# Shanmuk4622/RL-Project-Heist-Architect-Adversarial-Reinforcement-Learning-Framework-CSE4019

Measured on AMD Instinct MI355X. Metric: Solver env-steps/sec at 20×20, 4096 envs/GPU, 1/2/4/8 MI355X, higher is better.
Workload: dtype f64

## Files before the change

rl-project-heist-architect-adversarial-reinforcement-learning-framework-cse4019_amd/csrc/heist_env.hip:

```cpp
#include <type_traits>
#include <utility>

#include "heist_device.h"
#include "heist_fan_intervals.h"
#include "heist_trig.h"

#pragma clang fp contract(off)

namespace heist {

__constant__ double kSinCosTab[4 * HEIST_SINCOS_TAB_ROWS] = HEIST_SINCOS_TAB_INIT;
constexpr int kTabDoubles = 4 * HEIST_SINCOS_TAB_ROWS;

__device__ __forceinline__ int iabs_(int a) { return a < 0 ? -a : a; }
__device__ __forceinline__ int unpack_r(uint16_t v) { return v & 0xff; }
__device__ __forceinline__ int unpack_c(uint16_t v) { return v >> 8; }

__device__ __forceinline__ double py_mod360(double x) {
  if (x > 0.0 && x < 720.0) return x >= 360.0 ? x - 360.0 : x;
  double r = fmod(x, 360.0);
  if (r != 0.0) {
    if (r < 0.0) r += 360.0;
  } else {
    r = 0.0;
// ... 2441 lines not shown
  int hdr[4];
};

constexpr double kFanUnitsPerDeg = 4294967296.0 / 360.0;
struct IvlTable {
  uint32_t cut[kFanCuts];
  float2 dir[kFanCuts];
  uint8_t idx[368];
};
static_assert(sizeof(IvlTable) % 16 == 0, "copied in 16-byte words");
constexpr IvlTable make_ivl_table() {
  IvlTable t{};
  for (int j = 0; j < kFanCuts; ++j) {
    t.cut[j] = kFanCut[j];
    t.dir[j] = float2{kFanDir[j][0], kFanDir[j][1]};
  }
  for (int d = 0; d < 361; ++d) t.idx[d] = kFanIdx[d];
  return t;
}
__constant__ IvlTable kIvlTable = make_ivl_table();
constexpr size_t kLeanUnion = sizeof(LeanStage) > sizeof(IvlTable) ? sizeof(LeanStage) : sizeof(IvlTable);
struct LeanLds {
  uint8_t* grid;
  uint16_t* path;
  uint8_t* act;
  LeanStage* stg;
  IvlTable* ivl;
  uint4* icam;
  int32_t* icim;
  uint16_t* cone;
  uint16_t* rcone;
  uint8_t* gpl;
  float4* plane2;
};
__host__ __device__ constexpr int lean_gap(int R, int C) { return (R + 2 * kRing) * (C + 2 * kRing) <= 1024 ? 1024 : 2048; }
__host__ __device__ inline size_t lean_carve(unsigned char* smem, int R, int C, int mc, int mg, int mp, int K,
                                             LeanLds* L) {
  size_t o = 3 * (size_t)lean_gap(R, C);
  if (L) L->grid = smem + o;
  o += align16((size_t)R * C);
  if (L) L->path = reinterpret_cast<uint16_t*>(smem + o);
  o += align16(2 * (size_t)mg * mp);
  if (L) L->act = smem + o;
  o += align16((size_t)K);
  if (L) L->stg = reinterpret_cast<LeanStage*>(smem + o);
  if (L) L->ivl = reinterpret_cast<IvlTable*>(smem + o);
  o += align16(kLeanUnion);
  if (L) L->icam = reinterpret_cast<uint4*>(smem + o);
  o += 16 * (size_t)(mc > 0 ? mc : 1);
  if (L) L->icim = reinterpret_cast<int32_t*>(smem + o);
  o += align16(8 * (size_t)(mc > 0 ? mc : 1));
  if (L) L->cone = reinterpret_cast<uint16_t*>(smem + o);
  o += 64 * (size_t)(mg > 0 ? mg : 1);
  if (L) L->rcone = reinterpret_cast<uint16_t*>(smem + o);
  o += 64 * (size_t)(mg > 0 ? mg : 1);
  if (L) L->gpl = smem + o;
  o += align16((size_t)R * C);
  if (L) L->plane2 = reinterpret_cast<float4*>(smem + o);
  o += 4 * (size_t)R * C;
  return o;
}
static size_t lean_lds_bytes(const EnvParams& p, int K) {
  const size_t lean = align16(lean_carve(nullptr, p.R, p.C, p.max_cams, p.max_guards, p.max_path, K, nullptr)) +
                      (p.stamps ? 80 : 0);
  const size_t generic = step_multi_lds(p, K);
  return lean > generic ? lean : generic;
}


struct LeanGuard {
  uint32_t a, b, nslot;
  __device__ int idx() const { return (int)(a & 0xffu); }
  __device__ int step() const { return (int)((a >> 8) & 0xffu); }
  __device__ int len() const { return (int)((a >> 16) & 0xffu); }
  __device__ int hslot() const { return (int)(a >> 24); }
  __device__ uint32_t pos() const { return b & 0xffffu; }
  __device__ uint32_t pos0() const { return b >> 16; }
};

template <int D, bool REC>
__device__ __attribute__((noinline)) void lean_generic_body(EnvParams p, int K, const int64_t* __restrict__ actions,
                                                            obs_out_t<REC>* __restrict__ obs, float* __restrict__ rew,
                                                            double* __restrict__ rew64, uint8_t* __restrict__ done_out,
                                                            int8_t* __restrict__ status_out, int auto_reset,
                                                            unsigned char* smem, int e) {
  step_multi_body<1, D, false, 0, REC>(p, K, actions, obs, rew, rew64, done_out, status_out, auto_reset, smem, e);
}

template <int R_, int C_, bool STAMP = false, int NW = 1, bool REC = false>
__global__ __launch_bounds__(64 * NW) __attribute__((amdgpu_waves_per_eu(4))) void step_lean_kernel(
    EnvParams p, int K, const int64_t* __restrict__ actions, obs_out_t<REC>* __restrict__ obs, float* __restrict__ rew,
    double* __restrict__ rew64, uint8_t* __restrict__ done_out, int8_t* __restrict__ status_out, int auto_reset) {
  constexpr int D = lean_gap(R_, C_);
  constexpr int PC = C_ + 2 * kRing;
  constexpr int RC = R_ * C_;
  constexpr int N4 = RC / 4;
  constexpr int C4 = C_ / 4;
  constexpr int Q = (N4 + 63) / 64;
  constexpr int OFF0 = kRing * PC + kRing;
  static_assert((R_ + 2 * kRing) * PC <= D, "the padded planes fit the 1024-byte gap");
  static_assert(C_ % 4 == 0 && R_ <= 64 && C_ <= 32 && (R_ + 2 * kRing) * PC <= 2048, "lean kernel geometry");
  static_assert(NW == 1 || (NW == 2 && !STAMP && Q % 2 == 0), "two waves: the plain form, even Q");
  constexpr int QW = Q / NW;
  static_assert(!REC || !STAMP, "record output: the plain instances only");
  constexpr int NVIS = (RC + 31) / 32;
  constexpr int RW = (NVIS + 1 + 3) & ~3;
  constexpr int kStores = REC ? QW + 1 + 4 : 3 * QW + 4;
  extern __shared__ __align__(16) unsigned char smem[];
  const int e = block_env(p);
  if (p.prio_mode && p.dispatch_order) {
    const int pr = (int)((uint32_t)p.order[blockIdx.x] >> 24);
    if (pr == 3) __builtin_amdgcn_s_setprio(3);
    else if (pr == 2) __builtin_amdgcn_s_setprio(2);
    else if (pr == 1) __builtin_amdgcn_s_setprio(1);
  }
  const int lane = NW == 1 ? (int)threadIdx.x : (int)(threadIdx.x & 63u);
  const int wid = NW == 1 ? 0 : __builtin_amdgcn_readfirstlane((int)(threadIdx.x >> 6));
  const int tid = threadIdx.x;
  const int N = p.n_envs;
  const int mc = p.max_cams, mg = p.max_guards, n_slot = mc + mg, mp = p.max_path;
  const EnvBase eb = env_base(p, e);
  const FanTick* fan0 = p.fan + p.fan_base;

  EnvScalars s = p.scal[e];
  const int g = lane - mc;
  double heading = 0.0, speed = 0.0;
  uint32_t cam_rc = 0;
  LeanGuard gd{0u, 0u, 0u};
  const bool live_cam = lane < s.n_cams, live_guard = g >= 0 && g < s.n_guards;
  bool cached = false;
  double fovd = 0.0, su = 1.0;
  int32_t im_fx = 0;
  int cam_n = 0;
  bool ivl = false;
  {
    EmitterRaw rec;
    rec.a = make_uint4(0u, 0u, 0u, 0u);
    rec.b = rec.a;
    if (lane < n_slot) {
      const uint4* rs = lane < mc ? reinterpret_cast<const uint4*>(eb.cams + (uint32_t)lane)
                                  : reinterpret_cast<const uint4*>(eb.guards + (uint32_t)g);
      rec.a = rs[0];
      rec.b = rs[1];
    }
    const Cam cm = as_cam(rec);
    const Guard gr = as_guard(rec);
    heading = cm.heading;
    speed = cm.speed;
    cam_rc = (uint32_t)cm.row | ((uint32_t)cm.col << 8);
    cached = live_guard && gr.hslot != kUncached;
    gd.a = (uint32_t)(uint8_t)gr.idx | ((uint32_t)(uint8_t)gr.step << 8) | ((uint32_t)(uint8_t)gr.len << 16) |
           ((uint32_t)gr.hslot << 24);
    gd.b = (uint32_t)gr.pos | ((uint32_t)gr.pos0 << 16);
    gd.nslot = gr.nslot;
    const double f_heading = fan0->heading, f_speed = fan0->speed, f_fov = fan0->fov;
    const int f_rays = fan0->num_rays, f_range = fan0->range, f_uniq = fan0->n_uniq;
    const bool cam_ok = !live_cam || (py_mod360(cm.heading + cm.speed * 1.0) == f_heading && cm.speed == f_speed &&
                                      cm.fov == f_fov && cm.num_rays == f_rays && cm.range == f_range);
    const bool base_ok = p.ray_mode == 0 && !s.done && __ballot(live_guard && !cached) == 0ull;
    const bool fan_ok = p.fan_on && f_uniq >= 0 && f_range == kTieMaxRange && __ballot(!cam_ok) == 0ull;
    const double su_ = (cm.fov / (double)cm.num_rays) * kFanUnitsPerDeg;
    const bool ivl_cam = !live_cam || (cm.range == kTieMaxRange && cm.num_rays >= 1 && cm.fov > 0.0 &&
                                       cm.fov < 170.0 && su_ > 2.0 * (double)kFanMarginAxis + 8.0 &&
                                       su_ >= 2097153.0);
    ivl = base_ok && !fan_ok && p.interval_fans && __ballot(!ivl_cam) == 0ull;
    if (!base_ok || (!fan_ok && !ivl)) {
      if (NW == 2 && wid != 0) return;
      lean_generic_body<D, REC>(p, K, actions, obs, rew, rew64, done_out, status_out, auto_reset, smem, e);
      return;
    }
    if (live_cam) {
      fovd = cm.fov;
      su = su_;
      im_fx = (int32_t)__builtin_rint(4503599627370496.0 / su_);
      cam_n = cm.num_rays;
    }
  }

  LeanLds L;
  const size_t carved = lean_carve(smem, R_, C_, mc, mg, mp, K, &L);
  unsigned long long* st_acc = reinterpret_cast<unsigned long long*>(smem + align16(carved));
  unsigned long long st_last = 0, st_start = 0;
  if (STAMP && lane == 0) {
    st_start = st_last = __builtin_amdgcn_s_memtime();
    for (int j = 0; j < 9; ++j) st_acc[j] = 0;
  }
#define LEAN_STAMP(seg)                                        \
  do {                                                         \
    if (STAMP && lane == 0) {                                  \
      const unsigned long long now_ = __builtin_amdgcn_s_memtime(); \
      st_acc[(seg)] += now_ - st_last;                         \
      st_last = now_;                                          \
    }                                                          \
  } while (0)
  uint8_t* const wall = smem;
  uint8_t* const vis = smem + D;
  const uint32_t base = (uint32_t)(uintptr_t)smem;
  const uint32_t stg_a = (uint32_t)__builtin_amdgcn_readfirstlane((int)(uint32_t)(uintptr_t)L.stg);
  const uint32_t stc_a = (uint32_t)__builtin_amdgcn_readfirstlane((int)(uint32_t)(uintptr_t)L.cone);
  const uint32_t str_a = (uint32_t)__builtin_amdgcn_readfirstlane((int)(uint32_t)(uintptr_t)L.rcone);
  const uint32_t gpl_a = (uint32_t)__builtin_amdgcn_readfirstlane((int)(uint32_t)(uintptr_t)L.gpl);
  static_assert(RC % 16 == 0, "the packed guard plane is cleared in 16-byte words");
  {
    const uint32_t* g4 = reinterpret_cast<const uint32_t*>(p.grid + (size_t)e * RC);
    for (int i = tid; i < N4; i += 64 * NW) reinterpret_cast<uint32_t*>(L.grid)[i] = g4[i];
    const uint8_t* ss = p.stop + (size_t)e * p.stop_bytes;
    for (int i = tid; i < p.stop_bytes; i += 64 * NW) expand_stop(wall, i, ss[i]);
    const int vault = p.vr * C_ + p.vc, qv = vault >> 2;
    for (int q = tid; q < N4; q += 64 * NW) {
      float4 v = reinterpret_cast<const float4*>(p.plane0)[q];
      if (q == qv) patch4(v, vault & 3, p.vault_val);
      L.plane2[q] = v;
    }
  }
  for (int i = tid; i < mg * mp; i += 64 * NW) L.path[i] = eb.paths[i];
  for (int k = tid; k < K; k += 64 * NW) {
    const int64_t a = actions[(size_t)k * N + e];
    L.act[k] = (uint8_t)((a < 0 || a > 4) ? 0 : a);
  }
  __syncthreads();
  uint32_t vwall = 0;
  if (lane < R_)
    for (int c = 0; c < C_; ++c) vwall |= (uint32_t)wall[OFF0 + lane * PC + c] << c;

  auto dma_fan = [&](int k, bool wide) {
    const FanTick* f = fan0 + k;
    lds_dma16(f->off4 + lane, stg_a + (uint32_t)offsetof(LeanStage, off4));
    if (wide) lds_dma16(f->off4 + 64 + lane, stg_a + (uint32_t)offsetof(LeanStage, off4) + 1024u);
    lds_dma16(f->off2 + 2 * lane, stg_a + (uint32_t)offsetof(LeanStage, off2));
    if (lane == 0) lds_dma16(&f->num_rays, stg_a + (uint32_t)offsetof(LeanStage, hdr));
  };
  auto dma_cone = [&](int idx, int slot, uint32_t stage, int par) {
    if (cached) {
      const uint16_t* src = eb.cones + cone_off((uint32_t)g, (uint32_t)idx, (uint32_t)slot);
      const uint32_t dst = stage + (uint32_t)(par * 32 * mg) - 16u * (uint32_t)mc;
      lds_dma16(src, dst);
      lds_dma16(src + 8, dst + 16u * (uint32_t)mg);
    }
  };
  auto dma_next_cone = [&](int par) {
    int idx = gd.idx(), slot = gd.hslot();
    if (gd.len() >= 2) {
      idx += gd.step();
      if (idx >= gd.len()) idx -= gd.len();
      slot = (int)gd.nslot;
    }
    dma_cone(idx, slot, stc_a, par);
    if (auto_reset) dma_cone(0, slot, str_a, par);
  };
  if (wid == 0) dma_next_cone(0);
  if (ivl) {
    for (uint32_t o = 1024u * (uint32_t)wid; o < (uint32_t)sizeof(IvlTable); o += 1024u * NW)
      if (o + 16u * (uint32_t)lane < (uint32_t)sizeof(IvlTable))
        lds_dma16(reinterpret_cast<const unsigned char*>(&kIvlTable) + o + 16u * (uint32_t)lane, stg_a + o);
  } else if (wid == 0) {
    dma_fan(0, true);
  }
  asm volatile("s_waitcnt vmcnt(0)" ::: "memory");
  if (NW == 2) __syncthreads();

  const uint64_t cmask = __ballot(cached);
  auto stamp_cones = [&](const uint16_t* rows, int par) {
    if (lane < RC / 16) reinterpret_cast<uint4*>(L.gpl)[lane] = make_uint4(0u, 0u, 0u, 0u);
    const uint32_t gposv = gd.pos();
    for (int pass = 0; pass * 4 < mg; ++pass) {
      const int i = lane / 15, j = lane - 15 * i;
      const int gs = 4 * pass + i;
      const uint32_t gp = (uint32_t)__shfl((int)gposv, mc + (gs < mg ? gs : 0), 64);
      if (lane < 60 && gs < mg && ((cmask >> (mc + gs)) & 1u)) {
        const uint32_t bits = rows[par * 16 * mg + (j >> 3) * 8 * mg + 8 * gs + (j & 7)] & 0x7fffu;
        if (bits) {
          const uint32_t a0 = gpl_a + (unpack_r((uint16_t)gp) + j - kConeRange) * C_ +
                              (unpack_c((uint16_t)gp) - kConeRange);
          const uint32_t m = bits << (a0 & 3u);
          const uint32_t a = a0 & ~3u;
#pragma unroll
          for (int w = 0; w < 5; ++w) {
            const uint32_t nib = (m >> (4 * w)) & 15u;
            if (nib)
              __hip_atomic_fetch_or(reinterpret_cast<__attribute__((address_space(3))) uint32_t*>(a + 4 * w),
                                    __umul24(nib, 0x204081u) & 0x01010101u, __ATOMIC_RELAXED,
                                    __HIP_MEMORY_SCOPE_WORKGROUP);
          }
        }
      }
    }
  };
  auto march = [&](uint32_t corner, uint4 o4, uint2 o2) {
    const uint32_t ow[6] = {o4.x, o4.y, o4.z, o4.w, o2.x, o2.y};
    uint32_t a[12], w[12];
#pragma unroll
    for (int u = 0; u < 12; ++u) a[u] = corner + ((u & 1) ? (ow[u >> 1] >> 16) : (ow[u >> 1] & 0xffffu));
#pragma unroll
    for (int u = 0; u < 12; ++u) w[u] = lds_ld(a[u]);
    const uint32_t own0 = (ow[0] & 0xffffu) == (uint32_t)OFF0, own1 = (ow[0] >> 16) == (uint32_t)OFF0;
    uint32_t stop = 0;
#pragma unroll
    for (int u = 0; u < 12; ++u) {
      stop = u == 0 ? w[0] : or_b32(stop, w[u]);
      const uint32_t skip = u == 0 ? or_b32(stop, own0) : (u == 1 ? or_b32(stop, own1) : stop);
      lds_st(__umul24(skip, (uint32_t)D) + a[u] + D, 1);
    }
  };
  auto cast_fan = [&](int k, int n_uniq, int n_tie, int par, bool staged_wide) {
#pragma unroll
    for (int z = 0; z < D / 1024; ++z)
      reinterpret_cast<uint4*>(vis)[lane + 64 * z] = make_uint4(0u, 0u, 0u, 0u);
    const FanTick* f = fan0 + k;
    uint4 o4a = make_uint4(0u, 0u, 0u, 0u), o4b = o4a;
    uint2 o2a = make_uint2(0u, 0u), o2b = o2a;
    if (s.n_cams > 0) {
      const bool want_b = n_uniq > 64;
      o4a = L.stg->off4[lane];
      o2a = L.stg->off2[lane];
      if (want_b && staged_wide) {
        o4b = L.stg->off4[64 + lane];
        o2b = L.stg->off2[64 + lane];
      }
      if (want_b && !staged_wide) {
        o4b = f->off4[64 + lane];
        o2b = f->off2[64 + lane];
        asm volatile("" ::"v"(__builtin_bit_cast(u32x4_t, o4a)), "v"(__builtin_bit_cast(u32x2_t, o2a)),
                     "v"(__builtin_bit_cast(u32x4_t, o4b)), "v"(__builtin_bit_cast(u32x2_t, o2b)));
      }
    }
    if (k + 1 < K) {
      asm volatile("s_waitcnt lgkmcnt(0)" ::"v"(__builtin_bit_cast(u32x4_t, o4a)), "v"(__builtin_bit_cast(u32x2_t, o2a)),
                   "v"(__builtin_bit_cast(u32x4_t, o4b)), "v"(__builtin_bit_cast(u32x2_t, o2b))
                   : "memory");
      dma_fan(k + 1, n_uniq > 64);
    }
    if (s.n_cams > 0) {
      for (int m = 0; m < s.n_cams; ++m) {
        const uint32_t rcm = (uint32_t)__builtin_amdgcn_readlane((int)cam_rc, m);
        const uint32_t corner = base + (rcm & 0xffu) * PC + (rcm >> 8);
        if (lane < n_uniq) march(corner, o4a, o2a);
        if (lane + 64 < n_uniq) march(corner, o4b, o2b);
        for (int c0 = 128; c0 < n_uniq; c0 += 64)
          if (lane + c0 < n_uniq) march(corner, f->off4[lane + c0], f->off2[lane + c0]);
      }
      if (n_tie > 0) lean_tie_rays<D, PC>(smem, f, n_tie, cam_rc, s.n_cams, p.half_deg);
    }
    LEAN_STAMP(2);
    stamp_cones(L.cone, par);
  };
  auto wave_join = [&]() {
    if constexpr (NW == 2) asm volatile("s_waitcnt lgkmcnt(0)\n\ts_barrier" ::: "memory");
  };
  auto cast_ivl = [&](int par) {
    wave_join();
#pragma unroll
    for (int z = wid; z < D / 1024; z += NW)
      reinterpret_cast<uint4*>(vis)[lane + 64 * z] = make_uint4(0u, 0u, 0u, 0u);
    const double hmh = heading - fovd / 2.0;
    const double hu = (hmh < 0.0 ? hmh + 360.0 : hmh) * kFanUnitsPerDeg;
    const uint32_t h0v = hu >= 4294967295.0 ? 0xFFFFFFFFu : (uint32_t)hu;
    int cnt = 0, jb = 0;
    if (live_cam) {
      jb = (int)L.ivl->idx[__umulhi(h0v, 360u)] - 1;
      const uint64_t e64 = (uint64_t)h0v + (uint64_t)((double)cam_n * su) + (uint64_t)(kFanMarginAxis + 4);
      const int je = (int)L.ivl->idx[__umulhi((uint32_t)e64, 360u) + 1u] + kFanCuts * (int)(e64 >> 32);
      cnt = je - jb;
      L.icam[lane] = make_uint4(h0v, (uint32_t)jb, (uint32_t)cam_n | (cam_rc << 16), 0u);
      L.icim[lane] = im_fx;
    }
    int total = 0, jo_l = 0, end_l = 0;
    for (int m = 0; m < s.n_cams; ++m) {
      if (lane == m) jo_l = jb - total;
      total += __builtin_amdgcn_readlane(cnt, m);
      if (lane == m) end_l = total;
    }
    auto march_at = [&](uint32_t rc, float2 d) {
      const uint32_t row = rc & 0xffu, col = rc >> 8;
      const uint32_t own = base + (row + kRing) * PC + col + kRing;
      const float mx = __builtin_bit_cast(float, base + col + kRing), my = __builtin_bit_cast(float, row + kRing);
      march_fast<D, 2 * kTieMaxRange, false, false, true>(PC, own, d.x, d.y, mx, my, 2 * kTieMaxRange);
    };
    int mb = 0;
    wave_join();
    for (int q0 = 64 * wid; q0 < total; q0 += 64 * NW) {
      const int q = q0 + lane;
      while (__builtin_amdgcn_readlane(end_l, mb) <= q0) ++mb;
      int c = mb, jo = __builtin_amdgcn_readlane(jo_l, mb);
      for (int m = mb; m + 1 < s.n_cams; ++m) {
        const int em = __builtin_amdgcn_readlane(end_l, m);
        if (em >= q0 + 64) break;
        const int jo_m = __builtin_amdgcn_readlane(jo_l, m + 1);
        if (q >= em) {
          c = m + 1;
          jo = jo_m;
        }
      }
      int j = jo + q;
      j = j < 0 ? j + kFanCuts : (j >= kFanCuts ? j - kFanCuts : j);
      const uint4 cu = L.icam[c];
      const int im = L.icim[c];
      const int n = (int)(cu.z & 0xffffu);
      const int jn = j + 1 == kFanCuts ? 0 : j + 1;
      const uint32_t cut = L.ivl->cut[j], cutn = L.ivl->cut[jn];
      const float2 dj = L.ivl->dir[j];
      const int rel = (int)(cut - cu.x), reln = (int)(cutn - cu.x);
      const int mj = (cut & 0x3FFFFFFFu) ? kFanMarginTie : kFanMarginAxis;
      const int mn = (cutn & 0x3FFFFFFFu) ? kFanMarginTie : kFanMarginAxis;
      const int A = (__mulhi(rel + mj, im) >> 20) + 1;
      const int B = -(__mulhi(mj - rel, im) >> 20);
      const int Bn = -(__mulhi(mn - reln, im) >> 20);
      const int a0 = A > 0 ? A : 0;
      const bool act = q < total;
      const bool safe = act && a0 <= n && a0 < Bn;
      const bool near = act && B < A && B >= 0 && B <= n;
      if (__ballot(near)) {
        const double h_c = __shfl(hmh, c, 64), f_c = __shfl(fovd, c, 64);
        ivl_tie_rays<D, PC>(smem, near ? B : -1, h_c, f_c, n, cu.z >> 16, p.half_deg);
      }
      if (safe) march_at(cu.z >> 16, dj);
    }
    LEAN_STAMP(2);
    if (wid == 0) stamp_cones(L.cone, par);
    wave_join();
  };
  auto cast = [&](int k, int n_uniq, int n_tie, int par, bool staged_wide) {
    if (ivl) {
      cast_ivl(par);
    } else {
      wave_join();
      if (wid == 0) cast_fan(k, n_uniq, n_tie, par, staged_wide);
      wave_join();
    }
  };
  auto read_v1 = [&](uint32_t (&v1)[QW]) {
#pragma unroll
    for (int j = 0; j < QW; ++j) {
      const int q = lane + 64 * (wid * QW + j), qc = q < N4 ? q : N4 - 1, r = qc / C4;
      v1[j] = *reinterpret_cast<const uint32_t*>(vis + OFF0 + r * PC + 4 * (qc - r * C4)) |
              *reinterpret_cast<const uint32_t*>(L.gpl + 4 * qc);
    }
  };

  constexpr uint32_t kOOB = 0x40000000u;
  uint32_t vact = 0;
  bool wide = true;
  for (int k = 0; k < K; ++k) {
    const int par = k & 1;
    if ((k & 63) == 0) vact = k + lane < K ? L.act[k + lane] : 0u;
    asm volatile("s_waitcnt vmcnt(%0)" ::"i"(kStores) : "memory");
    int n_uniq = 0, n_tie = 0;
    if (!ivl && wid == 0) {
      const int2 h = *reinterpret_cast<const int2*>(&L.stg->hdr[2]);
      n_uniq = __builtin_amdgcn_readfirstlane(h.x);
      n_tie = __builtin_amdgcn_readfirstlane(h.y);
    }
    LEAN_STAMP(0);
    const bool staged_wide = wide;
    const bool frozen = s.done != 0;
    double reward = 0.0;
    int status = kAlreadyDone, curr = 0;
    if (!frozen) {
      const int a = __builtin_amdgcn_readlane((int)vact, k & 63);
      const int nr = s.pos_r + (a == 1 ? -1 : (a == 2 ? 1 : 0)), nc = s.pos_c + (a == 3 ? -1 : (a == 4 ? 1 : 0));
      if (nr >= 0 && nr < R_ && nc >= 0 && nc < C_ && !((__builtin_amdgcn_readlane((int)vwall, nr) >> nc) & 1)) {
        s.pos_r = nr;
        s.pos_c = nc;
      }
      status = kRunning;
      curr = iabs_(s.pos_r - p.vr) + iabs_(s.pos_c - p.vc);
      reward = p.r_step;
      reward += (double)(s.prev_dist - curr) * 0.1;
      if (curr <= 3 && s.initial_dist > 3) reward += 0.05 * (double)(3 - curr);
      s.prev_dist = curr;
      if (live_cam) heading = py_mod360(heading + speed * 1.0);
      if (live_guard && gd.len() >= 2) {
        int nidx = gd.idx() + gd.step();
        if (nidx >= gd.len()) nidx -= gd.len();
        const uint32_t np = L.path[__umul24((uint32_t)g, (uint32_t)mp) + (uint32_t)nidx];
        gd.a = (uint32_t)nidx | (gd.a & 0x00ffff00u) | (gd.nslot << 24);
        gd.b = np | (gd.b & 0xffff0000u);
      }
      if (cached && wid == 0) gd.nslot = L.cone[par * 16 * mg + 8 * mg + 8 * g + 7];
      if (k + 1 < K && wid == 0) dma_next_cone(par ^ 1);
      LEAN_STAMP(1);
      cast(k, n_uniq, n_tie, par, staged_wide);
      LEAN_STAMP(3);
    }
    wide = n_uniq > 64;
    uint32_t v1[QW];
    read_v1(v1);
    int done_now = s.done;
    LEAN_STAMP(4);
    if (!frozen) {
      bool seen;
      if constexpr (NW == 1) {
        const int sol = s.pos_r * C_ + s.pos_c, qs = sol >> 2;
        uint32_t vq = v1[0];
#pragma unroll
        for (int j = 1; j < Q; ++j) vq = (qs >> 6) == j ? v1[j] : vq;
        const uint32_t qv = (uint32_t)__builtin_amdgcn_readlane((int)vq, qs & 63);
        seen = ((qv >> (8 * (sol & 3))) & 0xffu) != 0u;
      } else {
        seen = (vis[OFF0 + s.pos_r * PC + s.pos_c] | L.gpl[s.pos_r * C_ + s.pos_c]) != 0;
      }
      if (seen) {
        s.detected = 1;
        reward += p.r_detect;
        s.done = 1;
        status = kDetected;
      }
      if (s.pos_r == p.vr && s.pos_c == p.vc) {
        s.vault_reached = 1;
        reward += p.r_vault;
        s.done = 1;
        status = kVaultReached;
      }
      s.tick += 1;
      if (s.tick >= p.max_steps) {
        s.done = 1;
        status = kTimeout;
        double frac = 1.0 - (double)curr / (double)(s.initial_dist > 1 ? s.initial_dist : 1);
        if (frac < 0.0) frac = 0.0;
        reward += frac * 2.0;
      }
      done_now = s.done;
    }
    LEAN_STAMP(5);
    if (auto_reset && done_now) {
      const bool moved = __ballot(live_guard && gd.pos() != gd.pos0()) != 0ull;
      reset_solver(p, s);
      if (live_guard) {
        gd.a &= ~0xffu;
        gd.b = (gd.b & 0xffff0000u) | gd.pos0();
      }
      if (cached && wid == 0) gd.nslot = L.rcone[par * 16 * mg + 8 * mg + 8 * g + 7];
      if (moved) {
        wave_join();
        if (wid == 0) stamp_cones(L.rcone, par);
        wave_join();
        read_v1(v1);
      }
      if (k + 1 < K && wid == 0) dma_next_cone(par ^ 1);
    }
    LEAN_STAMP(6);
    asm volatile("" ::: "memory");
    if constexpr (REC) {
      uint32_t* o = obs + ((size_t)k * N + e) * RW;
      const __amdgpu_buffer_rsrc_t rs = __builtin_amdgcn_make_buffer_rsrc(o, (short)0, 4 * RW, 0x00020000);
#pragma unroll
      for (int j = 0; j < QW; ++j) {
        const int q = lane + 64 * (wid * QW + j);
        uint32_t w = (q < N4 ? vis_nibble(v1[j]) : 0u) << (4 * (lane & 7));
        w = or8_lanes(w);
        const int wi = q >> 3;
        __builtin_amdgcn_raw_buffer_store_b32(w, rs, (lane & 7) == 0 && wi < NVIS ? 4 * wi : (int)kOOB, 0, 0);
      }
      __builtin_amdgcn_raw_buffer_store_b32(lane == 0 ? (uint32_t)s.pos_r | ((uint32_t)s.pos_c << 8) : 0u, rs,
                                            wid == 0 && lane < RW - NVIS ? 4 * (NVIS + lane) : (int)kOOB, 0, 0);
    } else {
      constexpr int pol = 2;
      float* o = obs + ((size_t)k * N + e) * 3 * RC;
      const __amdgpu_buffer_rsrc_t rs = __builtin_amdgcn_make_buffer_rsrc(o, (short)0, 12 * RC, 0x00020000);
      const int sol = s.pos_r * C_ + s.pos_c, qs = sol >> 2;
      const int vault = p.vr * C_ + p.vc;
  #pragma unroll
      for (int j = 0; j < QW; ++j) {
        const int q = lane + 64 * (wid * QW + j);
        const bool in = q < N4;
        const int qc = in ? q : N4 - 1;
        const uint32_t b = *reinterpret_cast<const uint32_t*>(L.grid + 4 * qc);
        obs_put(rs, pol, in ? 16 * q : (int)kOOB,
                make_float4((float)(b & 0xff) * 0.2f, (float)((b >> 8) & 0xff) * 0.2f,
                            (float)((b >> 16) & 0xff) * 0.2f, (float)(b >> 24) * 0.2f));
        const uint32_t v = v1[j];
        obs_put(rs, pol, in ? 16 * (N4 + q) : (int)kOOB,
                make_float4((float)(v & 0xff), (float)((v >> 8) & 0xff), (float)((v >> 16) & 0xff), (float)(v >> 24)));
        float4 c2 = L.plane2[qc];
        const bool pl = q == qs && sol != vault;
        const int m = sol & 3;
        c2.x = pl && m == 0 ? 1.0f + c2.x : c2.x;
        c2.y = pl && m == 1 ? 1.0f + c2.y : c2.y;
        c2.z = pl && m == 2 ? 1.0f + c2.z : c2.z;
        c2.w = pl && m == 3 ? 1.0f + c2.w : c2.w;
        obs_put(rs, pol, in ? 16 * (2 * N4 + q) : (int)kOOB, c2);
      }
    }
    const uint32_t ko = (uint32_t)((size_t)k * N + e);
    const int l0 = lane == 0 && wid == 0 ? 0 : (int)kOOB;
    __builtin_amdgcn_raw_buffer_store_b32(__builtin_bit_cast(uint32_t, (float)reward),
                                          __builtin_amdgcn_make_buffer_rsrc(rew + ko, (short)0, 4, 0x00020000), l0, 0, 0);
    __builtin_amdgcn_raw_buffer_store_b64(__builtin_bit_cast(u32x2_t, __builtin_bit_cast(uint64_t, reward)),
                                          __builtin_amdgcn_make_buffer_rsrc(rew64 ? rew64 + ko : rew64, (short)0,
                                                                            rew64 ? 8 : 0, 0x00020000),
                                          l0, 0, 0);
    __builtin_amdgcn_raw_buffer_store_b8((uint8_t)done_now,
                                         __builtin_amdgcn_make_buffer_rsrc(done_out + ko, (short)0, 1, 0x00020000), l0,
                                         0, 0);
    __builtin_amdgcn_raw_buffer_store_b8((uint8_t)(int8_t)status,
                                         __builtin_amdgcn_make_buffer_rsrc(status_out + ko, (short)0, 1, 0x00020000),
                                         l0, 0, 0);
    LEAN_STAMP(7);
  }
  if (STAMP && lane == 0) {
    unsigned long long* q = p.stamps + (size_t)e * p.multi_waves * 16;
    for (int j = 0; j < 9; ++j) q[j] = st_acc[j];
    q[9] = __builtin_amdgcn_s_memtime() - st_start;
    q[10] = st_start;
    q[11] = (unsigned)__builtin_amdgcn_s_getreg((31 << 11) | 4);
    q[12] = (unsigned)__builtin_amdgcn_s_getreg((31 << 11) | 20);
  }
#undef LEAN_STAMP
  if (wid != 0) return;
  if (lane == 0) p.scal[e] = s;
  if (live_cam) eb.cams[(uint32_t)lane].heading = heading;
  if (live_guard) {
    const uint4 c2 = reinterpret_cast<const uint4*>(eb.cones + cone_off(g, gd.idx(), gd.hslot()))[2];
    Guard* gp = eb.guards + (uint32_t)g;
    gp->heading = __builtin_bit_cast(double, ((uint64_t)c2.y << 32) | c2.x);
    gp->idx = (int16_t)gd.idx();
    gp->pos = (uint16_t)gd.pos();
    gp->hslot = (uint8_t)gd.hslot();
    gp->nslot = (uint8_t)gd.nslot;
  }
}

template <int W, int D>
__global__ __launch_bounds__(64 * W) __attribute__((amdgpu_waves_per_eu(kStepOcc))) void reset_kernel(EnvParams p, const uint8_t* __restrict__ mask,
                                                        float* __restrict__ obs) {
  constexpr int NT = 64 * W;
  extern __shared__ __align__(16) unsigned char smem[];
  const int e = block_env(p);
  const int t = threadIdx.x;
  if (mask && !mask[e]) return;
  const EnvLds L = carve<D>(smem, p.R, p.C, p.max_cams + p.max_guards, 0, W, p.max_guards);
  const EnvBase eb = env_base(p, e);
  EmitterRaw raw;
  prefetch<NT>(p, e, eb, L, raw);
  EnvScalars s = p.scal[e];
  const int mc = p.max_cams, n_slot = p.max_cams + p.max_guards;
  clear_vis<NT>(p, L);
  __syncthreads();
  reset_solver(p, s);
  Emit E;
  E.kind = -1;
  if (t < s.n_cams) {
    E = cam_emit(as_cam(raw));
  } else if (t >= mc && t - mc < s.n_guards) {
    Guard gd = as_guard(raw);
    gd.idx = 0;
    gd.pos = gd.pos0;
    Guard* gp = eb.guards + (uint32_t)(t - mc);
    gp->idx = 0;
    gp->pos = gd.pos0;
    if (gd.hslot != kUncached) {
      stage_guard_cone(p, e, L, t - mc, gd, false);
      gp->nslot = (uint8_t)L.cone[16 * (t - mc) + 15];
    }
    E = guard_emit(gd);
  }
  publish_emitters(L, E, n_slot);
  raycast_pass<NT, D>(p, e, smem, L, n_slot, mc);
  write_obs<NT>(p, e, s, L, 0, obs);
  if (t == 0) p.scal[e] = s;
}


__device__ __forceinline__ void write_stop_map(const EnvParams& p, int e, const uint8_t* g, int lane, int stride) {
  const int R = p.R, C = p.C, PC = C + 2 * kRing, nb = (R + 2 * kRing) * PC;
  uint8_t* stp = p.stop + (size_t)e * p.stop_bytes;
  for (int j = lane; j < p.stop_bytes; j += stride) {
    uint32_t bits = 0;
    for (int k = 0; k < 8; ++k) {
      const int i = 8 * j + k;
      const int pr = i / PC;
      const int r = pr - kRing, c = i - pr * PC - kRing;
      const bool out = i >= nb || (unsigned)r >= (unsigned)R || (unsigned)c >= (unsigned)C;
      if (out || g[r * C + c] == kWall) bits |= 1u << k;
    }
    stp[j] = (uint8_t)bits;
  }
}

int stop_map_bytes(int R, int C) { return (int)align16((size_t)(padded_bytes(R, C) + 7) / 8); }

__device__ bool bfs_wave(uint64_t pass, int sr, int sc, int gr, int gc) {
  const int lane = threadIdx.x & 63;
  if (sr == gr && sc == gc) return true;
  uint64_t reach = lane == sr ? (1ull << sc) : 0ull;
  const uint64_t goal = lane == gr ? (1ull << gc) : 0ull;
  for (int it = 0; it < kMaxDim * kMaxDim; ++it) {
    const uint64_t up = __shfl(reach, lane > 0 ? lane - 1 : 0);
    const uint64_t dn = __shfl(reach, lane < 63 ? lane + 1 : 63);
    const uint64_t nb = (reach | (reach << 1) | (reach >> 1) | (lane > 0 ? up : 0ull) | (lane < 63 ? dn : 0ull)) & pass;
    const uint64_t nxt = reach | nb;
    const bool hit = __any((nxt & goal) != 0ull);
    const bool grew = __any(nxt != reach);
    reach = nxt;
    if (hit) return true;
    if (!grew) return false;
  }
  return false;
}

__global__ __launch_bounds__(64) void set_layout_kernel(EnvParams p, int max_walls, const int32_t* __restrict__ wall_rc,
                                                         const int32_t* __restrict__ n_walls,
                                                         const double* __restrict__ cam_params,
                                                         const int32_t* __restrict__ n_cams,
                                                         const int32_t* __restrict__ guard_paths,
                                                         const int32_t* __restrict__ guard_meta,
                                                         const double* __restrict__ guard_fov,
                                                         const int32_t* __restrict__ n_guards,
                                                         const int32_t* __restrict__ budget,
                                                         const uint8_t* __restrict__ mask,
                                                         uint8_t* __restrict__ valid_out) {
  __shared__ uint8_t g[kMaxDim * kMaxDim];
  __shared__ int cnt[4];
  const int e = blockIdx.x;
  if (mask && !mask[e]) return;
  const int lane = threadIdx.x;
  const int R = p.R, C = p.C;
  for (int i = lane; i < p.RC; i += 64) {
    const int r = i / C, c = i - (i / C) * C;
    g[i] = (r == 0 || r == R - 1 || c == 0 || c == C - 1) ? kWall : kEmpty;
  }
  __syncthreads();
  if (lane == 0) {
    g[p.sr * C + p.sc] = kStart;
    g[p.vr * C + p.vc] = kVault;
    const int total = budget[e];
    int spent = 0, nw = 0, nc = 0, ng = 0;
    auto placeable = [&](int r, int c) {
      return r > 0 && r < R - 1 && c > 0 && c < C - 1 && g[r * C + c] == kEmpty;
    };
    const int wn = min(n_walls[e], max_walls);
    for (int i = 0; i < wn; ++i) {
      const int r = wall_rc[((size_t)e * max_walls + i) * 2], c = wall_rc[((size_t)e * max_walls + i) * 2 + 1];
      if (placeable(r, c) && total - spent >= 1) {
        spent += 1;
        g[r * C + c] = kWall;
        ++nw;
      }
    }
    const int cn = min(n_cams[e], p.max_cams);
    for (int i = 0; i < cn; ++i) {
      const double* cp = cam_params + ((size_t)e * p.max_cams + i) * 6;
      const int r = (int)cp[0], c = (int)cp[1];
      if (placeable(r, c) && total - spent >= 3) {
        spent += 3;
        Cam cm;
        cm.fov = cp[2]; cm.heading = cp[3]; cm.speed = cp[4];
        cm.row = (int16_t)r; cm.col = (int16_t)c; cm.range = (int16_t)cp[5];
        cm.num_rays = (int16_t)num_rays_for(cm.fov);
        p.cams[(size_t)e * p.max_cams + nc] = cm;
        g[r * C + c] = kCamera;
        ++nc;
      }
    }
    const int gn = min(n_guards[e], p.max_guards);
    for (int i = 0; i < gn; ++i) {
      const int32_t* gm = guard_meta + ((size_t)e * p.max_guards + i) * 3;
      const int len = min(gm[0], p.max_path);
      if (len > 0 && total - spent >= 5) {
        spent += 5;
        const int32_t* src = guard_paths + ((size_t)e * p.max_guards + i) * p.max_path * 2;
        uint16_t* dst = p.paths + ((size_t)e * p.max_guards + ng) * p.max_path;
        for (int k = 0; k < len; ++k) {
          const int pr = min(max(src[2 * k], 0), R - 1), pc = min(max(src[2 * k + 1], 0), C - 1);
          dst[k] = (uint16_t)pack_rc(pr, pc);
        }
        Guard gd;
        gd.fov = guard_fov[(size_t)e * p.max_guards + i];
        gd.heading = 0.0;
        gd.idx = 0;
        int st = gm[1] % len;
        if (st < 0) st += len;
        gd.step = (int16_t)st;
        gd.len = (int16_t)len;
        gd.range = (int16_t)gm[2];
        gd.num_rays = (int16_t)num_rays_for(gd.fov);
        gd.pos = dst[0];
        gd.pos0 = dst[0];
        gd.hslot = kUncached;
        gd.nslot = kUncached;
        p.guards[(size_t)e * p.max_guards + ng] = gd;
        g[unpack_r(dst[0]) * C + unpack_c(dst[0])] = kGuard;
        ++ng;
      }
    }
    cnt[0] = nw; cnt[1] = nc; cnt[2] = ng; cnt[3] = spent;
  }
  __syncthreads();
  uint64_t m = 0;
  if (lane < R)
    for (int c = 0; c < C; ++c)
      if (g[lane * C + c] != kWall) m |= 1ull << c;
  const bool ok = bfs_wave(m, p.sr, p.sc, p.vr, p.vc);
  uint8_t* dst = p.grid + (size_t)e * p.RC;
  for (int i = lane; i < p.RC; i += 64) dst[i] = g[i];
  write_stop_map(p, e, g, lane, 64);
  if (lane == 0) {
    EnvScalars* s = p.scal + e;
    s->n_walls = cnt[0];
    s->n_cams = cnt[1];
    s->n_guards = cnt[2];
    s->spent = cnt[3];
    valid_out[e] = ok ? 1 : 0;
  }
}

template <int D>
__global__ __launch_bounds__(64) void guard_cone_kernel(EnvParams p, const uint8_t* __restrict__ mask) {
  extern __shared__ __align__(16) unsigned char smem[];
  __shared__ double heads[kConeSlots];
  __shared__ uint8_t arr[kConePath];
  __shared__ int n_heads;
  const int e = blockIdx.x, g = blockIdx.y;
  const int lane = threadIdx.x;
  if (mask && !mask[e]) return;
  if (g >= p.scal[e].n_guards) return;
  Guard* gp = p.guards + (size_t)e * p.max_guards + g;
  const Guard gd = *gp;
  const int len = gd.len;
  if (!p.guard_cones || len < 1 || len > kConePath || gd.range < 0 || gd.range > kConeRange) return;
  const int R = p.R, C = p.C;
  const EnvLds L = carve<D>(smem, R, C, 1, kConePath, 1);
  const uint8_t* ss = p.stop + (size_t)e * p.stop_bytes;
  for (int i = lane; i < p.stop_bytes; i += 64) expand_stop(L.wall, i, ss[i]);
  if (lane < len) L.path[lane] = p.paths[((size_t)e * p.max_guards + g) * p.max_path + lane];
  __syncthreads();
  if (lane == 0) {
    int nh = 1;
    heads[0] = gd.heading;
    for (int j = 0; j < len; ++j) {
      int i0 = j - gd.step;
      if (i0 < 0) i0 += len;
      const int dr = unpack_r(L.path[j]) - unpack_r(L.path[i0]), dc = unpack_c(L.path[j]) - unpack_c(L.path[i0]);
      if (len < 2 || (dr == 0 && dc == 0)) {
        arr[j] = kUncached;
        continue;
      }
      const double h = guard_heading_after(p, dr, dc, 0.0);
      int k = 0;
      while (k < nh && heads[k] != h) ++k;
      if (k == nh) {
        if (nh == kConeSlots) {
          nh = 0;
// ... 585 lines not shown
```

Measured before the change: 805.7 million.

## Detect solver from camera LDS plus cached guard cone before stamping cones

Moves guard-cone stamping out of the cast functions and after the detection/reset logic. Detection now uses the camera visibility byte plus a direct lookup into the cached guard cone bitmask, so the view is read once and cones are stamped only once per step. This removes the second stamp and re-read that previously happened on reset when guards had moved. The trade-off is more complex ordering, with a risk of divergence when cones are not cached or when frozen environments skip stamping.

```diff
diff --git a/rl-project-heist-architect-adversarial-reinforcement-learning-framework-cse4019_amd/csrc/heist_env.hip b/rl-project-heist-architect-adversarial-reinforcement-learning-framework-cse4019_amd/csrc/heist_env.hip
--- a/rl-project-heist-architect-adversarial-reinforcement-learning-framework-cse4019_amd/csrc/heist_env.hip
+++ b/rl-project-heist-architect-adversarial-reinforcement-learning-framework-cse4019_amd/csrc/heist_env.hip
@@ -2767,7 +2767,7 @@
       lds_st(__umul24(skip, (uint32_t)D) + a[u] + D, 1);
     }
   };
-  auto cast_fan = [&](int k, int n_uniq, int n_tie, int par, bool staged_wide) {
+  auto cast_fan = [&](int k, int n_uniq, int n_tie, bool staged_wide) {
 #pragma unroll
     for (int z = 0; z < D / 1024; ++z)
       reinterpret_cast<uint4*>(vis)[lane + 64 * z] = make_uint4(0u, 0u, 0u, 0u);
@@ -2806,13 +2806,11 @@
       }
       if (n_tie > 0) lean_tie_rays<D, PC>(smem, f, n_tie, cam_rc, s.n_cams, p.half_deg);
     }
-    LEAN_STAMP(2);
-    stamp_cones(L.cone, par);
   };
   auto wave_join = [&]() {
     if constexpr (NW == 2) asm volatile("s_waitcnt lgkmcnt(0)\n\ts_barrier" ::: "memory");
   };
-  auto cast_ivl = [&](int par) {
+  auto cast_ivl = [&]() {
     wave_join();
 #pragma unroll
     for (int z = wid; z < D / 1024; z += NW)
@@ -2880,16 +2878,14 @@
       }
       if (safe) march_at(cu.z >> 16, dj);
     }
-    LEAN_STAMP(2);
-    if (wid == 0) stamp_cones(L.cone, par);
     wave_join();
   };
-  auto cast = [&](int k, int n_uniq, int n_tie, int par, bool staged_wide) {
+  auto cast = [&](int k, int n_uniq, int n_tie, bool staged_wide) {
     if (ivl) {
-      cast_ivl(par);
+      cast_ivl();
     } else {
       wave_join();
-      if (wid == 0) cast_fan(k, n_uniq, n_tie, par, staged_wide);
+      if (wid == 0) cast_fan(k, n_uniq, n_tie, staged_wide);
       wave_join();
     }
   };
@@ -2919,7 +2915,7 @@
     const bool staged_wide = wide;
     const bool frozen = s.done != 0;
     double reward = 0.0;
-    int status = kAlreadyDone, curr = 0;
+    int status = kAlreadyDone, curr = 0, done_now = s.done;
     if (!frozen) {
       const int a = __builtin_amdgcn_readlane((int)vact, k & 63);
       const int nr = s.pos_r + (a == 1 ? -1 : (a == 2 ? 1 : 0)), nc = s.pos_c + (a == 3 ? -1 : (a == 4 ? 1 : 0));
@@ -2942,28 +2938,17 @@
         gd.b = np | (gd.b & 0xffff0000u);
       }
       if (cached && wid == 0) gd.nslot = L.cone[par * 16 * mg + 8 * mg + 8 * g + 7];
-      if (k + 1 < K && wid == 0) dma_next_cone(par ^ 1);
       LEAN_STAMP(1);
-      cast(k, n_uniq, n_tie, par, staged_wide);
+      cast(k, n_uniq, n_tie, staged_wide);
+      LEAN_STAMP(2);
+      const uint32_t cam_sees = vis[OFF0 + s.pos_r * PC + s.pos_c];
+      uint32_t grow = 0;
+      const int sdr = s.pos_r - (int)unpack_r((uint16_t)gd.pos()) + kConeRange;
+      const int sdc = s.pos_c - (int)unpack_c((uint16_t)gd.pos()) + kConeRange;
+      if (cached && (unsigned)sdr <= 2u * kConeRange && (unsigned)sdc <= 2u * kConeRange)
+        grow = (L.cone[par * 16 * mg + (sdr >> 3) * 8 * mg + 8 * g + (sdr & 7)] & 0x7fffu) >> sdc;
+      const bool seen = (cam_sees | (uint32_t)(__ballot((grow & 1u) != 0u) != 0ull)) != 0u;
       LEAN_STAMP(3);
-    }
-    wide = n_uniq > 64;
-    uint32_t v1[QW];
-    read_v1(v1);
-    int done_now = s.done;
-    LEAN_STAMP(4);
-    if (!frozen) {
-      bool seen;
-      if constexpr (NW == 1) {
-        const int sol = s.pos_r * C_ + s.pos_c, qs = sol >> 2;
-        uint32_t vq = v1[0];
-#pragma unroll
-        for (int j = 1; j < Q; ++j) vq = (qs >> 6) == j ? v1[j] : vq;
-        const uint32_t qv = (uint32_t)__builtin_amdgcn_readlane((int)vq, qs & 63);
-        seen = ((qv >> (8 * (sol & 3))) & 0xffu) != 0u;
-      } else {
-        seen = (vis[OFF0 + s.pos_r * PC + s.pos_c] | L.gpl[s.pos_r * C_ + s.pos_c]) != 0;
-      }
       if (seen) {
         s.detected = 1;
         reward += p.r_detect;
@@ -2986,23 +2971,26 @@
       }
       done_now = s.done;
     }
-    LEAN_STAMP(5);
+    wide = n_uniq > 64;
+    LEAN_STAMP(4);
+    bool reset_moved = false;
     if (auto_reset && done_now) {
-      const bool moved = __ballot(live_guard && gd.pos() != gd.pos0()) != 0ull;
+      reset_moved = __ballot(live_guard && gd.pos() != gd.pos0()) != 0ull;
       reset_solver(p, s);
       if (live_guard) {
         gd.a &= ~0xffu;
         gd.b = (gd.b & 0xffff0000u) | gd.pos0();
       }
       if (cached && wid == 0) gd.nslot = L.rcone[par * 16 * mg + 8 * mg + 8 * g + 7];
-      if (moved) {
-        wave_join();
-        if (wid == 0) stamp_cones(L.rcone, par);
-        wave_join();
-        read_v1(v1);
-      }
-      if (k + 1 < K && wid == 0) dma_next_cone(par ^ 1);
-    }
+    }
+    if (!frozen && k + 1 < K && wid == 0) dma_next_cone(par ^ 1);
+    LEAN_STAMP(5);
+    if (!frozen) {
+      if (wid == 0) stamp_cones(reset_moved ? L.rcone : L.cone, par);
+      wave_join();
+    }
+    uint32_t v1[QW];
+    read_v1(v1);
     LEAN_STAMP(6);
     asm volatile("" ::: "memory");
     if constexpr (REC) {
```

Result: faster. 908.8 million, median of 6 (+12.8%).
